# fgnt/pb_chime5

Measured on AMD Instinct MI355X. Metric: utterance-seconds enhanced/sec/GPU (24ch, 20 EM iters), higher is better.
Workload: dtype f64

## Files before the change

pb_chime5_amd/csrc/cacgmm.hip:

```cpp
#include <algorithm>
#include <cmath>
#include <cstdlib>

#include "gss_internal.h"
#include "dense_wave.h"
#include "jacobi.h"

namespace {

#ifndef GSS_CHOL_PRIO
#define GSS_CHOL_PRIO 1
#endif
#ifndef GSS_ESTEP_PRIO
#define GSS_ESTEP_PRIO 1
#endif
constexpr int EM_TILE = 64;
constexpr int EM_TS = EM_TILE + 1;

enum { MODE_FIRST = 0, MODE_EM = 1, MODE_PREDICT = 2 };

__device__ __forceinline__ void set_progress_priority(int done, int total) {
    const int q4 = 4 * done / total;
    if (q4 <= 0) __builtin_amdgcn_s_setprio(3);
    else if (q4 == 1) __builtin_amdgcn_s_setprio(2);
    else if (q4 == 2) __builtin_amdgcn_s_setprio(1);
    else __builtin_amdgcn_s_setprio(0);
}

struct MsegPlan {
    int S, ntile, base, rem, maxseg;
};
__host__ __device__ __forceinline__ int mseg_begin(const MsegPlan &p, int slot) {
    return slot * p.base + (slot < p.rem ? slot : p.rem);
}
__host__ __device__ __forceinline__ int mseg_slot_of(const MsegPlan &p, int item) {
    const int head = p.rem * (p.base + 1);
    return item < head ? item / (p.base + 1) : p.rem + (item - head) / p.base;
}
__host__ __device__ __forceinline__ int mseg_count(const MsegPlan &p, int f) {
    return mseg_slot_of(p, f * p.ntile + p.ntile - 1) - mseg_slot_of(p, f * p.ntile) + 1;
}

struct EmArgs {
    const cplx *Y;
    const uint8_t *act;
    int64_t act_stride, act_fstride;
    const double *init;
    int64_t init_stride, init_fstride;
    const double *logdet;
    const double *pi;
// ... 2041 lines not shown
```

pb_chime5_amd/csrc/gss_api.hip:

```cpp
#include <cmath>
#include <cstdarg>
#include <cstdlib>
#include <cstring>
#include <mutex>

#include "gss_internal.h"

#define GSS_ENTER(ctx)                                   \
    if (!(ctx)) return GSS_ERR_INVALID;                  \
    GSS_HIP_CHECK((ctx), hipSetDevice((ctx)->device))
#define GSS_ENTER_VARIANTS(ctx) \
    GSS_ENTER(ctx);             \
    GSS_TRY(variant_refresh(ctx))
static int variant_refresh(gss_ctx *ctx);

static std::mutex g_error_lock;

int gss_fail(gss_ctx *ctx, int code, const char *fmt, ...) {
    char buf[1024];
    va_list ap;
    va_start(ap, fmt);
    vsnprintf(buf, sizeof(buf), fmt, ap);
    va_end(ap);
    if (ctx) {
        std::lock_guard<std::mutex> guard(g_error_lock);
        ctx->error = buf;
    }
    return code;
}

static thread_local std::string g_create_error;

namespace {
const char *const kVariantKeys[] = {
    "corr_ts", "corr_nw", "corr_blocked", "corr_p_tiles", "chol_diag_unfolded", "apply_ph",
    "apply_generic", "prof_detail", "corr_stg8", "corr_ksplit", "apply_gglobal", "wpe_halves",
    "em_wgs", "estep_wpb", "estep_lds", "mstep_prefetch_d", "mstep_tiled", "mstep_plan_min_d",
    "mstep_chunked", "mstep_slots", "force_eigh", "em_unfused", "em_l3_mb", "em_l3_fit_mb",
    "em_streams", "mstep_maxseg", "em4_cold_eigh", "mstep_generic"};
struct VariantTable {
    std::mutex lock;
    std::string text;
    bool parsed = false;
    std::map<std::string, int> values;
};
VariantTable &variant_table() {
    static VariantTable t;
    return t;
}
}

static int variant_refresh(gss_ctx *ctx) {
    const char *env = getenv("GSS_VARIANT");
    VariantTable &t = variant_table();
    std::lock_guard<std::mutex> guard(t.lock);
    if (t.parsed && t.text == (env ? env : "")) return GSS_OK;
    t.text = env ? env : "";
    t.parsed = true;
    t.values.clear();
// ... 1142 lines not shown
```

pb_chime5_amd/csrc/gss_internal.h:

```cpp
#pragma once
#include <hip/hip_runtime.h>

#include <cstdint>
#include <cstdio>
#include <map>
#include <string>
#include <vector>

#include "../../include/gss_hip.h"

typedef double2 cplx;

int gss_variant(const char *key, int dflt);
inline bool gss_variant_set(const char *key) { return gss_variant(key, 0) != 0; }

#if (defined(GSS_CORR_TRACE) || defined(GSS_WCOV_TRACE) || defined(GSS_EM4_TRACE) || \
     defined(GSS_CHOL_TRACE)) && !defined(GSS_EXPERIMENT_BUILD)
#error "trace instrumentation needs -DGSS_EXPERIMENT_BUILD=1 (tools/build_variant.sh)"
#endif

#define GSS_TINY 2.2250738585072014e-308

__device__ __forceinline__ cplx c_make(double r, double i) { return make_double2(r, i); }
__device__ __forceinline__ cplx c_add(cplx a, cplx b) { return make_double2(a.x + b.x, a.y + b.y); }
// ... 41 lines not shown
    const int lo = __builtin_amdgcn_update_dpp(0, (int)(unsigned)u, CTRL, ROW_MASK, BANK_MASK, true);
    const int hi = __builtin_amdgcn_update_dpp(0, (int)(unsigned)(u >> 32), CTRL, ROW_MASK, BANK_MASK, true);
    return __longlong_as_double(((unsigned long long)(unsigned)hi << 32) | (unsigned)lo);
}
__device__ __forceinline__ double wave_sum(double v) {
    double s = v + dpp_shifted<0x111, 0xf, 0xf>(v);
    s += dpp_shifted<0x112, 0xf, 0xf>(v);
    s += dpp_shifted<0x113, 0xf, 0xf>(v);
    s += dpp_shifted<0x114, 0xf, 0xe>(s);
    s += dpp_shifted<0x118, 0xf, 0xc>(s);
    s += dpp_shifted<0x142, 0xa, 0xf>(s);
    s += dpp_shifted<0x143, 0xc, 0xf>(s);
    const unsigned long long u = __double_as_longlong(s);
    const unsigned lo = __builtin_amdgcn_readlane((int)(unsigned)u, 63);
    const unsigned hi = __builtin_amdgcn_readlane((int)(unsigned)(u >> 32), 63);
    return __longlong_as_double(((unsigned long long)hi << 32) | lo);
}
__device__ __forceinline__ double wave_max(double v) {
#pragma unroll
    for (int o = 32; o > 0; o >>= 1) v = fmax(v, __shfl_xor(v, o, 64));
    return v;
}

__device__ __forceinline__ bool xcd_group_map(int nsub, int F, int &f, int &sub) {
    const int L = blockIdx.x;
    const int sg = L / (8 * nsub), rem = L - sg * 8 * nsub;
    sub = rem >> 3;
    f = sg * 8 + (rem & 7);
    return f < F;
}
static inline unsigned xcd_grid(int nsub, int F) { return (unsigned)(nsub * ((F + 7) / 8 * 8)); }

__host__ __device__ __forceinline__ int tri_index(int d1, int d2, int D) {
    return d1 * D - (d1 * (d1 - 1)) / 2 + (d2 - d1);
}
__host__ __device__ __forceinline__ int tri_count(int D) { return D * (D + 1) / 2; }

struct ProfEntry {
    std::string name;
    hipEvent_t start, stop;
};

struct gss_ctx {
    int device = 0;
    hipStream_t own_stream = nullptr;
    hipStream_t stream = nullptr;
// ... 139 lines not shown
```

pb_chime5_amd/csrc/wpe.hip:

```cpp
#include <algorithm>
#include <cmath>
#include <cstdlib>

#include "gss_internal.h"
#include <type_traits>
#include "dense_wave.h"

typedef double v4d __attribute__((ext_vector_type(4)));

namespace {

constexpr int POW_FRAMES = 256;
__global__ __launch_bounds__(POW_FRAMES) void wpe_power_kernel(const cplx *__restrict__ X,
                                                               int64_t T, int D, int psd_context,
                                                               double *__restrict__ raw,
                                                               double *__restrict__ w) {
    extern __shared__ __attribute__((aligned(16))) char smem[];
    double *ps = reinterpret_cast<double *>(smem);
    __shared__ double red[POW_FRAMES / 64];
    const int f = blockIdx.x, tid = threadIdx.x;
    const cplx *Xf = X + (int64_t)f * T * D;
    double *wout = w + (int64_t)f * T;
    double *wf = psd_context > 0 ? raw + (int64_t)f * T : wout;
    const int DP = D + 1;
    double mx = 0.0;
    for (int64_t t0 = 0; t0 < T; t0 += POW_FRAMES) {
        const int nfr = (int)min((int64_t)POW_FRAMES, T - t0);
        const int total = nfr * D;
        const cplx *src = Xf + t0 * D;
        __syncthreads();
        {
            constexpr int LB = 8;
            const int qf = POW_FRAMES / D, rf = POW_FRAMES - qf * D;
            int fr = tid / D, d = tid - fr * D;
            for (int base = tid; base < total; base += LB * POW_FRAMES) {
                cplx v[LB];
#pragma unroll
                for (int j = 0; j < LB; ++j) {
                    const int idx = base + j * POW_FRAMES;
                    v[j] = idx < total ? src[idx] : c_make(0.0, 0.0);
                }
#pragma unroll
                for (int j = 0; j < LB; ++j) {
                    if (base + j * POW_FRAMES < total) ps[fr * DP + d] = c_abs2(v[j]);
                    fr += qf;
                    d += rf;
                    if (d >= D) {
                        d -= D;
                        ++fr;
// ... 1036 lines not shown
                    }
                    nxim[it] = -xim[it];
#pragma unroll
                    for (int reg = 0; reg < 4; ++reg) {
                        const int rl = 16 * it + lk + 4 * reg, col = c0 + 16 * b + li;
                        if (rl < nb && col < D)
                            Z[(int64_t)(j0 + rl) * D + col] = c_make(xre[it][reg], xim[it][reg]);
                    }
                }
            }
            __syncthreads();
        }
    }
}

__global__ __launch_bounds__(256, 3) void chol_backsolve_kernel(const cplx *__restrict__ R,
                                                             cplx *__restrict__ P, int n, int D) {
    __shared__ cplx S[CH_NB * BS_LD];
    __shared__ cplx OP[BS_OPS];
    const int f = blockIdx.x;
    chol_backsolve_body(R + (int64_t)f * n * n, P + (int64_t)f * n * D, n, D, S, OP);
}

template <int TA, int NB, int NWV = 4, int WRAPS = 4, bool TAIL = true>
__global__ __launch_bounds__(64 * NWV) void wpe_apply_kernel(const cplx *__restrict__ Y,
                                                        const cplx *__restrict__ G, int F,
                                                        int64_t T, int D, int n, int c,
                                                        cplx *__restrict__ X) {
    constexpr int WAVE_FRAMES = 16 * TA, WG_FRAMES = NWV * WAVE_FRAMES;
    extern __shared__ __attribute__((aligned(16))) char smem[];
    cplx *S = reinterpret_cast<cplx *>(smem);
    const int DP = D | 1;
    int f, chunk;
    if (!xcd_group_map((int)((T + WG_FRAMES - 1) / WG_FRAMES), F, f, chunk)) return;
    const int64_t t0 = (int64_t)chunk * WG_FRAMES;
    const cplx *Yf = Y + (int64_t)f * T * D;
    const cplx *Gf = G + (int64_t)f * n * D;
    const int frames_lds = WG_FRAMES + c + 2;
    const int64_t fr0 = t0 - c;
    constexpr int PRE = 14, NT = 64 * NWV;
    const int total = frames_lds * D;
    for (int base = 0; base < total; base += NT * PRE) {
        cplx v[PRE];
#pragma unroll
        for (int j = 0; j < PRE; ++j) {
            const int idx = base + (int)threadIdx.x + NT * j;
            const int64_t fr = fr0 + idx / D;
            v[j] = c_make(0.0, 0.0);
            if (idx < total && fr >= 0 && fr < T) v[j] = Yf[fr0 * D + idx];
        }
#pragma unroll
        for (int j = 0; j < PRE; ++j) {
            const int idx = base + (int)threadIdx.x + NT * j;
            const int fl = idx / D, d = idx - fl * D;
            if (idx < total) S[fl * DP + d] = v[j];
        }
    }
    __syncthreads();
    const int wave = threadIdx.x >> 6, lane = threadIdx.x & 63;
    const int li = lane & 15, lk = lane >> 4;
    const int wf0 = wave * WAVE_FRAMES;
    if (t0 + wf0 >= T) return;
    v4d acc_re[TA][NB], acc_im[TA][NB], acc_t2[TA][NB];
#pragma unroll
    for (int a = 0; a < TA; ++a)
#pragma unroll
        for (int b = 0; b < NB; ++b) {
            acc_re[a][b] = (v4d){0.0, 0.0, 0.0, 0.0};
            acc_im[a][b] = (v4d){0.0, 0.0, 0.0, 0.0};
            acc_t2[a][b] = (v4d){0.0, 0.0, 0.0, 0.0};
        }
    const int ksteps = (n + 3) / 4;
    const int lds_last = frames_lds * DP - 1;
    int goff[NB], goff_max[NB];
#pragma unroll
    for (int b = 0; b < NB; ++b) {
        const int col = min(16 * b + li, D - 1);
        goff[b] = min(lk, n - 1) * D + col;
        goff_max[b] = (n - 1) * D + col;
    }
    auto load_g = [&](int, cplx (&g)[NB]) {
#pragma unroll
        for (int b = 0; b < NB; ++b) {
            g[b] = Gf[goff[b]];
            goff[b] = min(goff[b] + 4 * D, goff_max[b]);
        }
    };
    int rm = lk % D, lin = (lk / D) * DP + rm;
    int ubase[TA];
#pragma unroll
    for (int a = 0; a < TA; ++a) ubase[a] = (wf0 + 16 * a + li) * DP;
    auto load_u = [&](cplx (&u)[TA]) {
#pragma unroll
        for (int a = 0; a < TA; ++a) u[a] = S[min(ubase[a] + lin, lds_last)];
        rm += 4;
        lin += 4;
#pragma unroll
        for (int w = 0; w < WRAPS; ++w) {
            const bool wrap = rm >= D;
            rm -= wrap ? D : 0;
            lin += wrap ? DP - D : 0;
        }
    };
    auto step = [&](int ks, const cplx (&g)[NB], const cplx (&u)[TA]) {
        const bool ok = !TAIL || 4 * ks + lk < n;
        double ur[TA], ui[TA], gr[NB], gi[NB];
#pragma unroll
        for (int a = 0; a < TA; ++a) {
            ur[a] = ok ? u[a].x : 0.0;
            ui[a] = ok ? u[a].y : 0.0;
        }
#pragma unroll
        for (int b = 0; b < NB; ++b) {
            gr[b] = g[b].x;
            gi[b] = g[b].y;
        }
        double us[TA], gd[NB];
#pragma unroll
        for (int a = 0; a < TA; ++a) us[a] = ur[a] + ui[a];
#pragma unroll
        for (int b = 0; b < NB; ++b) gd[b] = gr[b] - gi[b];
#pragma unroll
        for (int a = 0; a < TA; ++a)
#pragma unroll
            for (int b = 0; b < NB; ++b) {
                acc_re[a][b] = __builtin_amdgcn_mfma_f64_16x16x4f64(ur[a], gr[b], acc_re[a][b], 0, 0, 0);
                acc_t2[a][b] = __builtin_amdgcn_mfma_f64_16x16x4f64(ui[a], gi[b], acc_t2[a][b], 0, 0, 0);
                acc_im[a][b] = __builtin_amdgcn_mfma_f64_16x16x4f64(us[a], gd[b], acc_im[a][b], 0, 0, 0);
            }
    };
    cplx g0[NB], g1[NB], u0[TA], u1[TA];
    load_g(0, g0);
    load_u(u0);
    for (int ks = 0; ks < ksteps; ks += 2) {
        load_g(ks + 1, g1);
        load_u(u1);
        __builtin_amdgcn_sched_barrier(0);
        step(ks, g0, u0);
        __builtin_amdgcn_sched_barrier(0);
        load_g(ks + 2, g0);
        load_u(u0);
        __builtin_amdgcn_sched_barrier(0);
        step(ks + 1, g1, u1);
        __builtin_amdgcn_sched_barrier(0);
    }
#pragma unroll
    for (int a = 0; a < TA; ++a)
#pragma unroll
        for (int b = 0; b < NB; ++b)
#pragma unroll
            for (int reg = 0; reg < 4; ++reg) {
                const int fl = wf0 + 16 * a + lk + 4 * reg;
                const int d = 16 * b + li;
                const int64_t t = t0 + fl;
                if (d < D && t < T) {
                    const cplx y = S[(fl + c) * DP + d];
                    const double pre = acc_re[a][b][reg] + acc_t2[a][b][reg];
                    const double pim = (acc_im[a][b][reg] - acc_re[a][b][reg]) + acc_t2[a][b][reg];
                    X[((int64_t)f * T + t) * D + d] = c_make(y.x - pre, y.y - pim);
                }
            }
}

template <int PH, int NT, bool GLDS = true, int PREW = 14, int PREG = 14>
__global__ __launch_bounds__(256) void wpe_apply_packed_kernel(const cplx *__restrict__ Y,
                                                               const cplx *__restrict__ G, int F,
                                                               int64_t T, int D, int n, int c,
                                                               cplx *__restrict__ X) {
    constexpr int WG_ROWS = 64, WG_FRAMES = PH * WG_ROWS;
    extern __shared__ __attribute__((aligned(16))) char smem[];
    const int DP = D | 1, DG = GLDS ? (D | 1) : D;
    const int frames_lds = WG_FRAMES + c + 2;
    cplx *S = reinterpret_cast<cplx *>(smem);
    cplx *Gl = S + (frames_lds * DP + frames_lds / PH + 1);
    int f, chunk;
    if (!xcd_group_map((int)((T + WG_FRAMES - 1) / WG_FRAMES), F, f, chunk)) return;
    const int64_t t0 = (int64_t)chunk * WG_FRAMES;
    const cplx *Yf = Y + (int64_t)f * T * D;
    const cplx *Gf = G + (int64_t)f * n * D;
    const int64_t fr0 = t0 - c;
    constexpr int NTHR = 256;
    {
        constexpr int PRE = PREW;
        const int total = frames_lds * D;
// ... 304 lines not shown
static int corr_tiles_pairs(int n, int D, int c, std::vector<CorrTile> &tiles) {
    for (int r0 = 0; r0 < n; r0 += 16)
        for (int c0 = r0; c0 < n; c0 += 32) tiles.push_back({r0, c0, 0, c0 + 16 < n ? 3 : 1});
    for (int r0 = 0; r0 < n; r0 += 32)
        for (int c0 = 0; c0 < D; c0 += 16) tiles.push_back({r0, c * D + c0, 1, r0 + 16 < n ? 5 : 1});
    std::stable_sort(tiles.begin(), tiles.end(), [](const CorrTile &x, const CorrTile &y) {
        return __builtin_popcount(x.mask) > __builtin_popcount(y.mask);
    });
    return (int)tiles.size();
}

static int corr_padf(int D, int ct) { return (ct + D - 1) / D + 1; }

size_t wpe_workspace_bytes(int F, int64_t T, int D, int taps, int delay) {
    const size_t n = (size_t)taps * D;
    size_t b = 0;
    b += 2 * align_up(sizeof(double) * (size_t)F * T);
    b += align_up(sizeof(cplx) * (size_t)F * n * n);
    b += align_up(sizeof(cplx) * (size_t)F * n * D);
    return b + 4096;
}

static int wpe_power_launch(gss_ctx *ctx, const cplx *cur, int F, int64_t T, int D,
                            int psd_context, double *raw, double *w) {
    const size_t pow_lds = sizeof(double) * POW_FRAMES * (D + 1);
    if (pow_lds > 64 * 1024)
        GSS_HIP_CHECK(ctx, hipFuncSetAttribute(reinterpret_cast<const void *>(wpe_power_kernel),
                                               hipFuncAttributeMaxDynamicSharedMemorySize,
                                               (int)pow_lds));
    hipLaunchKernelGGL(wpe_power_kernel, dim3(F), dim3(POW_FRAMES), pow_lds, ctx->stream,
                       cur, T, D, psd_context, raw, w);
    GSS_LAUNCH_CHECK(ctx, "wpe_power_kernel");
    return GSS_OK;
}

int wpe_inverse_power_run(gss_ctx *ctx, const cplx *Y, int F, int64_t T, int D, int psd_context,
                          double *w) {
    double *raw = psd_context > 0 ? arena_alloc_t<double>(ctx, (size_t)F * T) : nullptr;
    GSS_REQUIRE(ctx, raw || psd_context == 0, GSS_ERR_NOMEM, "wpe power workspace");
    return wpe_power_launch(ctx, Y, F, T, D, psd_context, raw, w);
}

int wpe_run(gss_ctx *ctx, const cplx *Y, int F, int64_t T, int D, int taps, int delay,
            int iterations, int psd_context, cplx *X, int part, int array_bins) {
    const int n = taps * D;
    const int c = delay + taps - 1;
    if (iterations == 0) {
        GSS_HIP_CHECK(ctx, hipMemsetAsync(ctx->status_dev + 2, 0, sizeof(int32_t), ctx->stream));
        if (X != Y)
            GSS_HIP_CHECK(ctx, hipMemcpyAsync(X, Y, sizeof(cplx) * (size_t)F * T * D,
                                              hipMemcpyDeviceToDevice, ctx->stream));
        return GSS_OK;
    }
    GSS_REQUIRE(ctx, X != Y, GSS_ERR_INVALID, "gss_wpe: X must not alias Y");
    double *w = arena_alloc_t<double>(ctx, (size_t)F * T);
    double *raw = psd_context > 0 ? arena_alloc_t<double>(ctx, (size_t)F * T) : nullptr;
    cplx *R = arena_alloc_t<cplx>(ctx, (size_t)F * n * n);
    cplx *P = arena_alloc_t<cplx>(ctx, (size_t)F * n * D);
    GSS_REQUIRE(ctx, w && (raw || psd_context == 0) && R && P, GSS_ERR_NOMEM, "wpe workspace");

    std::vector<CorrTile> tiles;
    const int sub16 = (n + 15) / 16;
    int corr_ts = sub16 * (sub16 + 1) / 2 + sub16 * ((D + 15) / 16) <= CORR_FINE_MAX_SUBTILES ? 1 : 2;
    bool corr_pairs = false;
    if (const int e = gss_variant("corr_ts", 0)) {
        corr_ts = e == 1 ? 1 : 2;
        corr_pairs = e == 3;
    }
    const int ntiles = corr_pairs ? corr_tiles_pairs(n, D, c, tiles) : corr_tiles(n, D, c, 16 * corr_ts, tiles);
    constexpr int tm16 = 16, tn16 = 16;
    std::vector<UpdTile> upd;
    std::vector<int> upd_start, upd_count, upd_j0, upd_k, upd_ndiag;
    const bool fold_diag = !gss_variant_set("chol_diag_unfolded");
    {
        const int nblk = (n + CH_NB - 1) / CH_NB;
        for (int J = 0; J < nblk; ++J) {
            upd_start.push_back((int)upd.size());
            const int rs = (J + 1) * CH_NB;
            const bool narrow = J % 2 == 0;
            const int r_end = narrow ? std::min(rs + CH_NB, n) : n;
            const int d_end = std::min(rs + CH_NB, n);
            for (int r0 = rs; r0 < d_end; r0 += tm16)
// ... 55 lines not shown
                   : corr_ts == 1 ? (corr_nw == 2 ? wpe_corr_kernel<1, 2> : wpe_corr_kernel<1, 4>)
                                  : (corr_nw == 2 ? wpe_corr_kernel<2, 2> : wpe_corr_kernel<2, 4>);
    size_t corr_lds = sizeof(cplx) * (size_t)(CORR_KT + c + padf) * D + sizeof(double) * CORR_KT;
    const int ksplit_forced = gss_variant("corr_ksplit", 0);
    int cus = 0;
    if (array_bins > 0)
        GSS_HIP_CHECK(ctx, hipDeviceGetAttribute(&cus, hipDeviceAttributeMultiprocessorCount, ctx->device));
    const bool arrays_single_waves = array_bins > 0 && (int64_t)ntiles * array_bins >= 4LL * 16 * cus;
    const bool corr_split = ksplit_forced ? ksplit_forced != 1 : !arrays_single_waves;
    const int corr_ks = (corr_ts == 1 && corr_nw == 1 && corr_split)
                            ? (ksplit_forced == 2 ? 2 : 4) : 1;
    using corr_fn_t = void (*)(const cplx *, const double *, int, int64_t, int, int, int, int,
                               const CorrTile *, int, cplx *, cplx *);
    corr_fn_t ksplit_fn = nullptr;
    if (corr_ks > 1) {
        ksplit_fn = corr_stg5 ? (corr_ks == 2 ? wpe_corr_ksplit_kernel<2, 5> : wpe_corr_ksplit_kernel<4, 5>)
                              : (corr_ks == 2 ? wpe_corr_ksplit_kernel<2, 8> : wpe_corr_ksplit_kernel<4, 8>);
        corr_lds = std::max(corr_lds * corr_ks, sizeof(cplx) * 256 * (size_t)(corr_ks - 1));
    }
    const size_t panel_lds = sizeof(cplx) * UDP_SIZE + sizeof(double) * CH_NB;
    constexpr int apply_ta = 2;
    constexpr int apply_nwv = 4;
    const int apply_frames = 16 * apply_ta * apply_nwv;
    auto apply_fn = D <= 16 ? wpe_apply_kernel<apply_ta, 1> : wpe_apply_kernel<apply_ta, 2>;
    if (D >= 4 && !gss_variant_set("apply_generic")) {
        if (n % 8 == 0)
            apply_fn = D <= 16 ? wpe_apply_kernel<apply_ta, 1, 4, 1, false>
                               : wpe_apply_kernel<apply_ta, 2, 4, 1, false>;
        else
            apply_fn = D <= 16 ? wpe_apply_kernel<apply_ta, 1, 4, 1, true>
                               : wpe_apply_kernel<apply_ta, 2, 4, 1, true>;
    }
    const size_t apply_lds = sizeof(cplx) * (size_t)(apply_frames + c + 2) * (D | 1);
    int apply_ph = 1, apply_nt = (D + 15) / 16;
    size_t packed_lds = 0;
    {
        const int ph_env = gss_variant("apply_ph", 0);
        bool ph_env_taken = ph_env <= 1;
        double best = (double)((D + 15) / 16) * n;
        for (int ph = 2; ph <= 4; ++ph) {
            if (ph_env > 0 && ph != ph_env) continue;
            const int nt = (ph * D + 15) / 16;
            if (nt > 3 || D < 2) continue;
            const double cost = (double)nt * (n + (ph - 1) * D) / ph;
            const int fl = 64 * ph + c + 2;
            const size_t lds = sizeof(cplx) * ((size_t)fl * (D | 1) + fl / ph + 1 + (size_t)(n + 1) * (D | 1));
            if (lds > (ph_env == ph ? 160 : 64) * 1024) continue;
            if (cost < 0.75 * best || ph_env == ph) {
                ph_env_taken = ph_env_taken || ph_env == ph;
                best = cost;
                apply_ph = ph;
                apply_nt = nt;
                packed_lds = lds;
            }
        }
// ... 18 lines not shown
        packed_lds = sizeof(cplx) * ((size_t)fl * (D | 1) + fl / 2 + 1);
        packed_fn = wpe_apply_packed_kernel<2, 3, false>;
    } else
    if (apply_ph > 1) {
        static const apply_packed_t table[3][3] = {
            {wpe_apply_packed_kernel<2, 1>, wpe_apply_packed_kernel<2, 2>, wpe_apply_packed_kernel<2, 3>},
            {wpe_apply_packed_kernel<3, 1>, wpe_apply_packed_kernel<3, 2>, wpe_apply_packed_kernel<3, 3>},
            {wpe_apply_packed_kernel<4, 1>, wpe_apply_packed_kernel<4, 2>, wpe_apply_packed_kernel<4, 3>}};
        packed_fn = table[apply_ph - 2][apply_nt - 1];
        static const apply_packed_t table_small[3][3] = {
            {wpe_apply_packed_kernel<2, 1, true, 4, 1>, wpe_apply_packed_kernel<2, 2, true, 4, 1>, wpe_apply_packed_kernel<2, 3, true, 4, 1>},
            {wpe_apply_packed_kernel<3, 1, true, 4, 1>, wpe_apply_packed_kernel<3, 2, true, 4, 1>, wpe_apply_packed_kernel<3, 3, true, 4, 1>},
            {wpe_apply_packed_kernel<4, 1, true, 4, 1>, wpe_apply_packed_kernel<4, 2, true, 4, 1>, wpe_apply_packed_kernel<4, 3, true, 4, 1>}};
        if ((64 * apply_ph + c + 2) * D <= 4 * 256 && n * D <= 256 && !gss_variant_set("apply_generic"))
            packed_fn = table_small[apply_ph - 2][apply_nt - 1];
        if (packed_lds > 64 * 1024)
            GSS_HIP_CHECK(ctx, hipFuncSetAttribute(reinterpret_cast<const void *>(packed_fn),
                                                   hipFuncAttributeMaxDynamicSharedMemorySize,
                                                   (int)packed_lds));
    }
    GSS_REQUIRE(ctx, corr_lds <= 160 * 1024 && apply_lds <= 160 * 1024, GSS_ERR_UNSUPPORTED,
                "wpe: taps=%d D=%d needs more LDS than a CU has", taps, D);
    if (apply_lds > 64 * 1024)
        GSS_HIP_CHECK(ctx, hipFuncSetAttribute(reinterpret_cast<const void *>(apply_fn),
                                               hipFuncAttributeMaxDynamicSharedMemorySize,
                                               (int)apply_lds));
    if (corr_lds > 64 * 1024)
        GSS_HIP_CHECK(ctx, hipFuncSetAttribute(reinterpret_cast<const void *>(corr_fn),
                                               hipFuncAttributeMaxDynamicSharedMemorySize,
                                               (int)corr_lds));
    const int corr_pieces = (int)(((size_t)(CORR_KT + c + padf) * D + 63) / 64);
    const size_t corr_dma_lds = 2 * (sizeof(cplx) * 64 * (size_t)corr_pieces + sizeof(double) * CORR_KT);
    const bool corr_persist = corr_ts == 2 && (int64_t)T * D * 16 < (1LL << 31) &&
                              corr_dma_lds <= 80 * 1024;
    if (corr_persist && !nw_forced) corr_nw = 4;
    const bool corr_blocked = corr_persist && gss_variant_set("corr_blocked");
    auto corr_persist_fn = corr_blocked ? (corr_nw == 2 ? wpe_corr_persist_kernel<2, true>
                                                        : wpe_corr_persist_kernel<4, true>)
                                        : (corr_nw == 2 ? wpe_corr_persist_kernel<2>
                                                        : wpe_corr_persist_kernel<4>);
    CorrQueue corr_queue{(ntiles + corr_nw - 1) / corr_nw, 0};
    int corr_slots = 0;
    if (corr_persist) {
        for (int g = 0; g < corr_queue.ngroups; ++g)
            if (__builtin_popcount(tiles[g * corr_nw].mask) >= 3) corr_queue.gh = g + 1;
        if (corr_dma_lds > 64 * 1024)
            GSS_HIP_CHECK(ctx, hipFuncSetAttribute(reinterpret_cast<const void *>(corr_persist_fn),
                                                   hipFuncAttributeMaxDynamicSharedMemorySize,
                                                   (int)corr_dma_lds));
        int per_cu = 0, cus = 0;
        GSS_HIP_CHECK(ctx, hipOccupancyMaxActiveBlocksPerMultiprocessor(
                               &per_cu, reinterpret_cast<const void *>(corr_persist_fn), 64 * corr_nw,
                               corr_dma_lds));
        GSS_HIP_CHECK(ctx, hipDeviceGetAttribute(&cus, hipDeviceAttributeMultiprocessorCount, ctx->device));
        corr_slots = std::min(std::max(per_cu, 1) * cus, corr_queue.ngroups * F);
    }

    for (int it = 0; it < iterations; ++it) {
        const cplx *cur = it == 0 ? Y : X;
        {
            GSS_PROF(ctx, "wpe_power");
            GSS_TRY(wpe_power_launch(ctx, cur, F, T, D, psd_context, raw, w));
        }
        if (corr_persist) {
            GSS_HIP_CHECK(ctx, hipMemsetAsync(corr_counters, 0, 8 * 16 * sizeof(int), ctx->stream));
            GSS_PROF(ctx, "wpe_corr");
            hipLaunchKernelGGL(corr_persist_fn, dim3(corr_slots), dim3(64 * corr_nw), corr_dma_lds,
                               ctx->stream, Y, w, F, T, D, n, c, corr_pieces, tiles_dev, ntiles,
                               corr_queue, corr_counters, R, P);
            GSS_LAUNCH_CHECK(ctx, "wpe_corr_persist_kernel");
        } else {
            GSS_PROF(ctx, "wpe_corr");
            if (ksplit_fn)
                hipLaunchKernelGGL(ksplit_fn, dim3(xcd_grid(ntiles, F)), dim3(64 * corr_ks), corr_lds,
                                   ctx->stream, Y, w, F, T, D, n, c, padf, tiles_dev, ntiles, R, P);
            else
                hipLaunchKernelGGL(corr_fn, dim3(xcd_grid((ntiles + corr_nw - 1) / corr_nw, F)),
                                   dim3(64 * corr_nw), corr_lds,
                                   ctx->stream, Y, w, F, T, D, n, c, padf, tiles_dev, ntiles, R, P);
            GSS_LAUNCH_CHECK(ctx, "wpe_corr_kernel");
        }
        {
            const int nblk = (n + CH_NB - 1) / CH_NB;
            const bool detail = gss_variant_set("prof_detail");
            static const char *trsm_names[] = {"wpe_chol_trsm_J0", "wpe_chol_trsm_J1", "wpe_chol_trsm_J2",
// ... 21 lines not shown
                    const int ndiag = upd_ndiag[J];
                    const dim3 g((ndiag > 0 ? (F + 7) / 8 * 8 : 0) +
                                 xcd_grid((nupd - ndiag + UPD_WAVES - 1) / UPD_WAVES, F)), b(64 * UPD_WAVES);
                    const UpdTile *tl = upd_dev + upd_start[J];
                    hipLaunchKernelGGL((chol_update_kernel<1, 1, true>), g, b, 0, ctx->stream, R, P, F, n, D, upd_j0[J],
                                       std::min(upd_k[J], n - upd_j0[J]), tl, nupd, ndiag,
                                       (J + 1) * CH_NB, zero_pivots);
                    GSS_LAUNCH_CHECK(ctx, "chol_update_kernel");
                }
            }
            {
                GSS_PROF(ctx, "wpe_backsolve");
                hipLaunchKernelGGL(chol_backsolve_kernel, dim3(F), dim3(256), 0, ctx->stream, R, P, n,
                                   D);
                GSS_LAUNCH_CHECK(ctx, "chol_backsolve_kernel");
            }
        }
        {
            GSS_PROF(ctx, "wpe_apply");
            if (packed_fn) {
                const int wg_frames = 64 * apply_ph;
                hipLaunchKernelGGL(packed_fn, dim3(xcd_grid((int)((T + wg_frames - 1) / wg_frames), F)),
                                   dim3(256), packed_lds, ctx->stream, Y, P, F, T, D, n, c, X);
            } else {
                hipLaunchKernelGGL(apply_fn,
                                   dim3(xcd_grid((int)((T + apply_frames - 1) / apply_frames), F)),
                                   dim3(64 * apply_nwv), apply_lds, ctx->stream, Y, P, F, T, D, n, c, X);
            }
            GSS_LAUNCH_CHECK(ctx, "wpe_apply_kernel");
        }
    }
    if (part < 0)
        GSS_HIP_CHECK(ctx, hipMemcpyAsync(ctx->status_host + 2, zero_pivots, sizeof(int32_t),
                                          hipMemcpyDeviceToHost, ctx->stream));
    return GSS_OK;
}


int wpe_copy_zero_pivots(gss_ctx *ctx) {
    if (!ctx->wpe_tiles) return GSS_OK;
    const int32_t *zero_pivots =
        reinterpret_cast<const int32_t *>(reinterpret_cast<const CorrTile *>(ctx->wpe_tiles) + 1024 + 4096);
    GSS_HIP_CHECK(ctx, hipMemcpyAsync(ctx->status_host + 2, zero_pivots, sizeof(int32_t),
                                      hipMemcpyDeviceToHost, ctx->stream));
    return GSS_OK;
}

int selftest_mfma_run(gss_ctx *ctx) {
    double *out = nullptr;
    GSS_HIP_CHECK(ctx, hipMalloc(reinterpret_cast<void **>(&out), sizeof(double) * 256));
// ... 17 lines not shown
```

Before: 1091.

## Fuse WPE power computation into apply kernel and add persistent run-based apply

```diff
diff --git a/pb_chime5_amd/csrc/cacgmm.hip b/pb_chime5_amd/csrc/cacgmm.hip
--- a/pb_chime5_amd/csrc/cacgmm.hip
+++ b/pb_chime5_amd/csrc/cacgmm.hip
@@ -18,14 +18,6 @@
 constexpr int EM_TS = EM_TILE + 1;
 
 enum { MODE_FIRST = 0, MODE_EM = 1, MODE_PREDICT = 2 };
-
-__device__ __forceinline__ void set_progress_priority(int done, int total) {
-    const int q4 = 4 * done / total;
-    if (q4 <= 0) __builtin_amdgcn_s_setprio(3);
-    else if (q4 == 1) __builtin_amdgcn_s_setprio(2);
-    else if (q4 == 2) __builtin_amdgcn_s_setprio(1);
-    else __builtin_amdgcn_s_setprio(0);
-}
 
 struct MsegPlan {
     int S, ntile, base, rem, maxseg;
diff --git a/pb_chime5_amd/csrc/gss_api.hip b/pb_chime5_amd/csrc/gss_api.hip
--- a/pb_chime5_amd/csrc/gss_api.hip
+++ b/pb_chime5_amd/csrc/gss_api.hip
@@ -35,6 +35,7 @@
 const char *const kVariantKeys[] = {
     "corr_ts", "corr_nw", "corr_blocked", "corr_p_tiles", "chol_diag_unfolded", "apply_ph",
     "apply_generic", "prof_detail", "corr_stg8", "corr_ksplit", "apply_gglobal", "wpe_halves",
+    "power_pass", "apply_grid",
     "em_wgs", "estep_wpb", "estep_lds", "mstep_prefetch_d", "mstep_tiled", "mstep_plan_min_d",
     "mstep_chunked", "mstep_slots", "force_eigh", "em_unfused", "em_l3_mb", "em_l3_fit_mb",
     "em_streams", "mstep_maxseg", "em4_cold_eigh", "mstep_generic"};
diff --git a/pb_chime5_amd/csrc/gss_internal.h b/pb_chime5_amd/csrc/gss_internal.h
--- a/pb_chime5_amd/csrc/gss_internal.h
+++ b/pb_chime5_amd/csrc/gss_internal.h
@@ -87,6 +87,20 @@
     return v;
 }
 
+__device__ __forceinline__ void set_progress_priority(int done, int total) {
+    const int q4 = 4 * done / total;
+    if (q4 <= 0) __builtin_amdgcn_s_setprio(3);
+    else if (q4 == 1) __builtin_amdgcn_s_setprio(2);
+    else if (q4 == 2) __builtin_amdgcn_s_setprio(1);
+    else __builtin_amdgcn_s_setprio(0);
+}
+
+__device__ __forceinline__ void wave_lds_sync() {
+    __builtin_amdgcn_fence(__ATOMIC_RELEASE, "wavefront");
+    __builtin_amdgcn_wave_barrier();
+    __builtin_amdgcn_fence(__ATOMIC_ACQUIRE, "wavefront");
+}
+
 __device__ __forceinline__ bool xcd_group_map(int nsub, int F, int &f, int &sub) {
     const int L = blockIdx.x;
     const int sg = L / (8 * nsub), rem = L - sg * 8 * nsub;
diff --git a/pb_chime5_amd/csrc/wpe.hip b/pb_chime5_amd/csrc/wpe.hip
--- a/pb_chime5_amd/csrc/wpe.hip
+++ b/pb_chime5_amd/csrc/wpe.hip
@@ -11,6 +11,7 @@
 namespace {
 
 constexpr int POW_FRAMES = 256;
+template <bool FROM_RAW = false>
 __global__ __launch_bounds__(POW_FRAMES) void wpe_power_kernel(const cplx *__restrict__ X,
                                                                int64_t T, int D, int psd_context,
                                                                double *__restrict__ raw,
@@ -21,10 +22,17 @@
     const int f = blockIdx.x, tid = threadIdx.x;
     const cplx *Xf = X + (int64_t)f * T * D;
     double *wout = w + (int64_t)f * T;
-    double *wf = psd_context > 0 ? raw + (int64_t)f * T : wout;
+    double *wf = psd_context > 0 || FROM_RAW ? raw + (int64_t)f * T : wout;
     const int DP = D + 1;
     double mx = 0.0;
-    for (int64_t t0 = 0; t0 < T; t0 += POW_FRAMES) {
+    if (FROM_RAW && psd_context == 0) {
+        for (int64_t t = tid; t < T; t += POW_FRAMES) {
+            const double p = wf[t];
+            wout[t] = p;
+            mx = fmax(mx, p);
+        }
+    }
+    for (int64_t t0 = 0; !FROM_RAW && t0 < T; t0 += POW_FRAMES) {
         const int nfr = (int)min((int64_t)POW_FRAMES, T - t0);
         const int total = nfr * D;
         const cplx *src = Xf + t0 * D;
@@ -1107,11 +1115,147 @@
     chol_backsolve_body(R + (int64_t)f * n * n, P + (int64_t)f * n * D, n, D, S, OP);
 }
 
-template <int TA, int NB, int NWV = 4, int WRAPS = 4, bool TAIL = true>
+template <int TA, int NB, int WRAPS, bool TAIL, bool POWER, bool SHARED>
+__device__ __forceinline__ void apply_wave_tile(const cplx *S, double *Q, int frames_lds, int wf0,
+                                                bool active, const cplx *__restrict__ Gf, int f,
+                                                int64_t t0, int64_t T, int D, int DP, int n, int c,
+                                                cplx *__restrict__ X, double *__restrict__ raw,
+                                                int lane) {
+    constexpr int WAVE_FRAMES = 16 * TA;
+    const int li = lane & 15, lk = lane >> 4;
+    v4d acc_re[TA][NB], acc_im[TA][NB], acc_t2[TA][NB];
+#pragma unroll
+    for (int a = 0; a < TA; ++a)
+#pragma unroll
+        for (int b = 0; b < NB; ++b) {
+            acc_re[a][b] = (v4d){0.0, 0.0, 0.0, 0.0};
+            acc_im[a][b] = (v4d){0.0, 0.0, 0.0, 0.0};
+            acc_t2[a][b] = (v4d){0.0, 0.0, 0.0, 0.0};
+        }
+    const int ksteps = active ? (n + 3) / 4 : 0;
+    const int lds_last = frames_lds * DP - 1;
+    int goff[NB], goff_max[NB];
+#pragma unroll
+    for (int b = 0; b < NB; ++b) {
+        const int col = min(16 * b + li, D - 1);
+        goff[b] = min(lk, n - 1) * D + col;
+        goff_max[b] = (n - 1) * D + col;
+    }
+    auto load_g = [&](int, cplx (&g)[NB]) {
+#pragma unroll
+        for (int b = 0; b < NB; ++b) {
+            g[b] = Gf[goff[b]];
+            goff[b] = min(goff[b] + 4 * D, goff_max[b]);
+        }
+    };
+    int rm = lk % D, lin = (lk / D) * DP + rm;
+    int ubase[TA];
+#pragma unroll
+    for (int a = 0; a < TA; ++a) ubase[a] = (wf0 + 16 * a + li) * DP;
+    auto load_u = [&](cplx (&u)[TA]) {
+#pragma unroll
+        for (int a = 0; a < TA; ++a) u[a] = S[min(ubase[a] + lin, lds_last)];
+        rm += 4;
+        lin += 4;
+#pragma unroll
+        for (int w = 0; w < WRAPS; ++w) {
+            const bool wrap = rm >= D;
+            rm -= wrap ? D : 0;
+            lin += wrap ? DP - D : 0;
+        }
+    };
+    auto step = [&](int ks, const cplx (&g)[NB], const cplx (&u)[TA]) {
+        const bool ok = !TAIL || 4 * ks + lk < n;
+        double ur[TA], ui[TA], gr[NB], gi[NB];
+#pragma unroll
+        for (int a = 0; a < TA; ++a) {
+            ur[a] = ok ? u[a].x : 0.0;
+            ui[a] = ok ? u[a].y : 0.0;
+        }
+#pragma unroll
+        for (int b = 0; b < NB; ++b) {
+            gr[b] = g[b].x;
+            gi[b] = g[b].y;
+        }
+        double us[TA], gd[NB];
+#pragma unroll
+        for (int a = 0; a < TA; ++a) us[a] = ur[a] + ui[a];
+#pragma unroll
+        for (int b = 0; b < NB; ++b) gd[b] = gr[b] - gi[b];
+#pragma unroll
+        for (int a = 0; a < TA; ++a)
+#pragma unroll
+            for (int b = 0; b < NB; ++b) {
+                acc_re[a][b] = __builtin_amdgcn_mfma_f64_16x16x4f64(ur[a], gr[b], acc_re[a][b], 0, 0, 0);
+                acc_t2[a][b] = __builtin_amdgcn_mfma_f64_16x16x4f64(ui[a], gi[b], acc_t2[a][b], 0, 0, 0);
+                acc_im[a][b] = __builtin_amdgcn_mfma_f64_16x16x4f64(us[a], gd[b], acc_im[a][b], 0, 0, 0);
+            }
+    };
+    cplx g0[NB], g1[NB], u0[TA], u1[TA];
+    load_g(0, g0);
+    load_u(u0);
+    for (int ks = 0; ks < ksteps; ks += 2) {
+        load_g(ks + 1, g1);
+        load_u(u1);
+        __builtin_amdgcn_sched_barrier(0);
+        step(ks, g0, u0);
+        __builtin_amdgcn_sched_barrier(0);
+        load_g(ks + 2, g0);
+        load_u(u0);
+        __builtin_amdgcn_sched_barrier(0);
+        step(ks + 1, g1, u1);
+        __builtin_amdgcn_sched_barrier(0);
+    }
+    double pw[TA][NB][4];
+#pragma unroll
+    for (int a = 0; a < TA; ++a)
+#pragma unroll
+        for (int b = 0; b < NB; ++b)
+#pragma unroll
+            for (int reg = 0; reg < 4; ++reg) {
+                const int fl = wf0 + 16 * a + lk + 4 * reg;
+                const int d = 16 * b + li;
+                const int64_t t = t0 + fl;
+                pw[a][b][reg] = 0.0;
+                if (d < D && t < T) {
+                    const cplx y = S[(fl + c) * DP + d];
+                    const double pre = acc_re[a][b][reg] + acc_t2[a][b][reg];
+                    const double pim = (acc_im[a][b][reg] - acc_re[a][b][reg]) + acc_t2[a][b][reg];
+                    const cplx x = c_make(y.x - pre, y.y - pim);
+                    if (POWER)
+                        pw[a][b][reg] = c_abs2(x);
+                    else
+                        X[((int64_t)f * T + t) * D + d] = x;
+                }
+            }
+    if (POWER) {
+        static_assert(WAVE_FRAMES <= 64, "one lane per frame of a wave");
+        if (SHARED) __syncthreads(); else wave_lds_sync();
+#pragma unroll
+        for (int a = 0; a < TA; ++a)
+#pragma unroll
+            for (int b = 0; b < NB; ++b)
+#pragma unroll
+                for (int reg = 0; reg < 4; ++reg) {
+                    const int d = 16 * b + li;
+                    if (d < D) Q[(16 * a + lk + 4 * reg) * DP + d] = pw[a][b][reg];
+                }
+        if (SHARED) __syncthreads(); else wave_lds_sync();
+        const int64_t t = t0 + wf0 + lane;
+        if (lane < WAVE_FRAMES && t < T) {
+            double p = 0.0;
+            for (int d = 0; d < D; ++d) p += Q[lane * DP + d];
+            raw[(int64_t)f * T + t] = p / (double)D;
+        }
+    }
+}
+
+template <int TA, int NB, int NWV = 4, int WRAPS = 4, bool TAIL = true, bool POWER = false>
 __global__ __launch_bounds__(64 * NWV) void wpe_apply_kernel(const cplx *__restrict__ Y,
                                                         const cplx *__restrict__ G, int F,
                                                         int64_t T, int D, int n, int c,
-                                                        cplx *__restrict__ X) {
+                                                        cplx *__restrict__ X,
+                                                        double *__restrict__ raw) {
     constexpr int WAVE_FRAMES = 16 * TA, WG_FRAMES = NWV * WAVE_FRAMES;
     extern __shared__ __attribute__((aligned(16))) char smem[];
     cplx *S = reinterpret_cast<cplx *>(smem);
@@ -1143,108 +1287,71 @@
     }
     __syncthreads();
     const int wave = threadIdx.x >> 6, lane = threadIdx.x & 63;
-    const int li = lane & 15, lk = lane >> 4;
     const int wf0 = wave * WAVE_FRAMES;
-    if (t0 + wf0 >= T) return;
-    v4d acc_re[TA][NB], acc_im[TA][NB], acc_t2[TA][NB];
-#pragma unroll
-    for (int a = 0; a < TA; ++a)
-#pragma unroll
-        for (int b = 0; b < NB; ++b) {
-            acc_re[a][b] = (v4d){0.0, 0.0, 0.0, 0.0};
-            acc_im[a][b] = (v4d){0.0, 0.0, 0.0, 0.0};
-            acc_t2[a][b] = (v4d){0.0, 0.0, 0.0, 0.0};
-        }
-    const int ksteps = (n + 3) / 4;
-    const int lds_last = frames_lds * DP - 1;
-    int goff[NB], goff_max[NB];
-#pragma unroll
-    for (int b = 0; b < NB; ++b) {
-        const int col = min(16 * b + li, D - 1);
-        goff[b] = min(lk, n - 1) * D + col;
-        goff_max[b] = (n - 1) * D + col;
-    }
-    auto load_g = [&](int, cplx (&g)[NB]) {
-#pragma unroll
-        for (int b = 0; b < NB; ++b) {
-            g[b] = Gf[goff[b]];
-            goff[b] = min(goff[b] + 4 * D, goff_max[b]);
-        }
-    };
-    int rm = lk % D, lin = (lk / D) * DP + rm;
-    int ubase[TA];
-#pragma unroll
-    for (int a = 0; a < TA; ++a) ubase[a] = (wf0 + 16 * a + li) * DP;
-    auto load_u = [&](cplx (&u)[TA]) {
-#pragma unroll
-        for (int a = 0; a < TA; ++a) u[a] = S[min(ubase[a] + lin, lds_last)];
-        rm += 4;
-        lin += 4;
-#pragma unroll
-        for (int w = 0; w < WRAPS; ++w) {
-            const bool wrap = rm >= D;
-            rm -= wrap ? D : 0;
-            lin += wrap ? DP - D : 0;
-        }
-    };
-    auto step = [&](int ks, const cplx (&g)[NB], const cplx (&u)[TA]) {
-        const bool ok = !TAIL || 4 * ks + lk < n;
-        double ur[TA], ui[TA], gr[NB], gi[NB];
-#pragma unroll
-        for (int a = 0; a < TA; ++a) {
-            ur[a] = ok ? u[a].x : 0.0;
-            ui[a] = ok ? u[a].y : 0.0;
-        }
-#pragma unroll
-        for (int b = 0; b < NB; ++b) {
-            gr[b] = g[b].x;
-            gi[b] = g[b].y;
-        }
-        double us[TA], gd[NB];
-#pragma unroll
-        for (int a = 0; a < TA; ++a) us[a] = ur[a] + ui[a];
-#pragma unroll
-        for (int b = 0; b < NB; ++b) gd[b] = gr[b] - gi[b];
-#pragma unroll
-        for (int a = 0; a < TA; ++a)
-#pragma unroll
-            for (int b = 0; b < NB; ++b) {
-                acc_re[a][b] = __builtin_amdgcn_mfma_f64_16x16x4f64(ur[a], gr[b], acc_re[a][b], 0, 0, 0);
-                acc_t2[a][b] = __builtin_amdgcn_mfma_f64_16x16x4f64(ui[a], gi[b], acc_t2[a][b], 0, 0, 0);
-                acc_im[a][b] = __builtin_amdgcn_mfma_f64_16x16x4f64(us[a], gd[b], acc_im[a][b], 0, 0, 0);
-            }
-    };
-    cplx g0[NB], g1[NB], u0[TA], u1[TA];
-    load_g(0, g0);
-    load_u(u0);
-    for (int ks = 0; ks < ksteps; ks += 2) {
-        load_g(ks + 1, g1);
-        load_u(u1);
-        __builtin_amdgcn_sched_barrier(0);
-        step(ks, g0, u0);
-        __builtin_amdgcn_sched_barrier(0);
-        load_g(ks + 2, g0);
-        load_u(u0);
-        __builtin_amdgcn_sched_barrier(0);
-        step(ks + 1, g1, u1);
-        __builtin_amdgcn_sched_barrier(0);
-    }
-#pragma unroll
-    for (int a = 0; a < TA; ++a)
-#pragma unroll
-        for (int b = 0; b < NB; ++b)
-#pragma unroll
-            for (int reg = 0; reg < 4; ++reg) {
-                const int fl = wf0 + 16 * a + lk + 4 * reg;
-                const int d = 16 * b + li;
-                const int64_t t = t0 + fl;
-                if (d < D && t < T) {
-                    const cplx y = S[(fl + c) * DP + d];
-                    const double pre = acc_re[a][b][reg] + acc_t2[a][b][reg];
-                    const double pim = (acc_im[a][b][reg] - acc_re[a][b][reg]) + acc_t2[a][b][reg];
-                    X[((int64_t)f * T + t) * D + d] = c_make(y.x - pre, y.y - pim);
+    const bool active = t0 + wf0 < T;
+    if (!POWER && !active) return;
+    apply_wave_tile<TA, NB, WRAPS, TAIL, POWER, true>(S, reinterpret_cast<double *>(smem) + wf0 * DP,
+                                                      frames_lds, wf0, active, Gf, f, t0, T, D, DP, n,
+                                                      c, X, raw, lane);
+}
+
+template <int TA, int NB, int NWV = 4, int WRAPS = 4, bool TAIL = true, bool POWER = false>
+__global__ __launch_bounds__(64 * NWV) void wpe_apply_runs_kernel(const cplx *__restrict__ Y,
+                                                             const cplx *__restrict__ G, int ntile,
+                                                             int nitems, int64_t T, int D, int n,
+                                                             int c, cplx *__restrict__ X,
+                                                             double *__restrict__ raw) {
+    constexpr int WAVE_FRAMES = 16 * TA;
+    extern __shared__ __attribute__((aligned(16))) char smem[];
+    const int DP = D | 1;
+    const int wave = __builtin_amdgcn_readfirstlane((int)threadIdx.x >> 6), lane = threadIdx.x & 63;
+    const int frames_lds = WAVE_FRAMES + c + 2;
+    cplx *S = reinterpret_cast<cplx *>(smem) + wave * frames_lds * DP;
+    const int nwaves = (int)gridDim.x * NWV, w = (int)blockIdx.x * NWV + wave;
+    const int run = nitems / nwaves, rem = nitems - run * nwaves;
+    const int beg = w * run + min(w, rem), end = beg + run + (w < rem ? 1 : 0);
+    const int total = frames_lds * D;
+    const int qf = 64 / D, rf = 64 - qf * D;
+    const int fl0 = lane / D, d0 = lane - fl0 * D;
+    int f = beg / ntile, tile = beg - f * ntile;
+    for (int item = beg; item < end; ++item) {
+        set_progress_priority(item - beg, end - beg);
+        const int64_t t0 = (int64_t)tile * WAVE_FRAMES;
+        const int64_t fr0 = t0 - c;
+        const cplx *src = Y + ((int64_t)f * T + fr0) * D;
+        constexpr int PRE = NB == 1 ? 6 : 18;
+        int fl = fl0, d = d0;
+        for (int base = 0; base < total; base += 64 * PRE) {
+            cplx v[PRE];
+            int so[PRE];
+#pragma unroll
+            for (int j = 0; j < PRE; ++j) {
+                const int idx = base + lane + 64 * j;
+                const int64_t fr = fr0 + fl;
+                v[j] = c_make(0.0, 0.0);
+                if (idx < total && fr >= 0 && fr < T) v[j] = src[idx];
+                so[j] = idx < total ? fl * DP + d : -1;
+                fl += qf;
+                d += rf;
+                if (d >= D) {
+                    d -= D;
+                    ++fl;
                 }
             }
+#pragma unroll
+            for (int j = 0; j < PRE; ++j)
+                if (so[j] >= 0) S[so[j]] = v[j];
+        }
+        wave_lds_sync();
+        apply_wave_tile<TA, NB, WRAPS, TAIL, POWER, false>(S, reinterpret_cast<double *>(S), frames_lds,
+                                                           0, true, G + (int64_t)f * n * D, f, t0, T,
+                                                           D, DP, n, c, X, raw, lane);
+        wave_lds_sync();
+        if (++tile == ntile) {
+            tile = 0;
+            ++f;
+        }
+    }
 }
 
 template <int PH, int NT, bool GLDS = true, int PREW = 14, int PREG = 14>
@@ -1595,13 +1702,19 @@
 }
 
 static int wpe_power_launch(gss_ctx *ctx, const cplx *cur, int F, int64_t T, int D,
-                            int psd_context, double *raw, double *w) {
+                            int psd_context, double *raw, double *w, bool from_raw = false) {
+    if (from_raw) {
+        hipLaunchKernelGGL(wpe_power_kernel<true>, dim3(F), dim3(POW_FRAMES), 0, ctx->stream,
+                           cur, T, D, psd_context, raw, w);
+        GSS_LAUNCH_CHECK(ctx, "wpe_power_kernel");
+        return GSS_OK;
+    }
     const size_t pow_lds = sizeof(double) * POW_FRAMES * (D + 1);
     if (pow_lds > 64 * 1024)
-        GSS_HIP_CHECK(ctx, hipFuncSetAttribute(reinterpret_cast<const void *>(wpe_power_kernel),
+        GSS_HIP_CHECK(ctx, hipFuncSetAttribute(reinterpret_cast<const void *>(wpe_power_kernel<false>),
                                                hipFuncAttributeMaxDynamicSharedMemorySize,
                                                (int)pow_lds));
-    hipLaunchKernelGGL(wpe_power_kernel, dim3(F), dim3(POW_FRAMES), pow_lds, ctx->stream,
+    hipLaunchKernelGGL(wpe_power_kernel<false>, dim3(F), dim3(POW_FRAMES), pow_lds, ctx->stream,
                        cur, T, D, psd_context, raw, w);
     GSS_LAUNCH_CHECK(ctx, "wpe_power_kernel");
     return GSS_OK;
@@ -1612,6 +1725,31 @@
     double *raw = psd_context > 0 ? arena_alloc_t<double>(ctx, (size_t)F * T) : nullptr;
     GSS_REQUIRE(ctx, raw || psd_context == 0, GSS_ERR_NOMEM, "wpe power workspace");
     return wpe_power_launch(ctx, Y, F, T, D, psd_context, raw, w);
+}
+
+using apply_fn_t = void (*)(const cplx *, const cplx *, int, int64_t, int, int, int, cplx *, double *);
+template <int TA, bool POWER>
+static apply_fn_t pick_apply(int D, int form) {
+    if (form == 1)
+        return D <= 16 ? wpe_apply_kernel<TA, 1, 4, 1, false, POWER> : wpe_apply_kernel<TA, 2, 4, 1, false, POWER>;
+    if (form == 2)
+        return D <= 16 ? wpe_apply_kernel<TA, 1, 4, 1, true, POWER> : wpe_apply_kernel<TA, 2, 4, 1, true, POWER>;
+    return D <= 16 ? wpe_apply_kernel<TA, 1, 4, 4, true, POWER> : wpe_apply_kernel<TA, 2, 4, 4, true, POWER>;
+}
+
+constexpr int kApplyGridDefault = 1;
+using apply_runs_fn_t = void (*)(const cplx *, const cplx *, int, int, int64_t, int, int, int, cplx *,
+                                 double *);
+template <int TA, bool POWER>
+static apply_runs_fn_t pick_apply_runs(int D, int form) {
+    if (form == 1)
+        return D <= 16 ? wpe_apply_runs_kernel<TA, 1, 4, 1, false, POWER>
+                       : wpe_apply_runs_kernel<TA, 2, 4, 1, false, POWER>;
+    if (form == 2)
+        return D <= 16 ? wpe_apply_runs_kernel<TA, 1, 4, 1, true, POWER>
+                       : wpe_apply_runs_kernel<TA, 2, 4, 1, true, POWER>;
+    return D <= 16 ? wpe_apply_runs_kernel<TA, 1, 4, 4, true, POWER>
+                   : wpe_apply_runs_kernel<TA, 2, 4, 4, true, POWER>;
 }
 
 int wpe_run(gss_ctx *ctx, const cplx *Y, int F, int64_t T, int D, int taps, int delay,
@@ -1627,10 +1765,11 @@
     }
     GSS_REQUIRE(ctx, X != Y, GSS_ERR_INVALID, "gss_wpe: X must not alias Y");
     double *w = arena_alloc_t<double>(ctx, (size_t)F * T);
-    double *raw = psd_context > 0 ? arena_alloc_t<double>(ctx, (size_t)F * T) : nullptr;
+    double *raw = psd_context > 0 || iterations > 1 ? arena_alloc_t<double>(ctx, (size_t)F * T) : nullptr;
     cplx *R = arena_alloc_t<cplx>(ctx, (size_t)F * n * n);
     cplx *P = arena_alloc_t<cplx>(ctx, (size_t)F * n * D);
-    GSS_REQUIRE(ctx, w && (raw || psd_context == 0) && R && P, GSS_ERR_NOMEM, "wpe workspace");
+    GSS_REQUIRE(ctx, w && (raw || (psd_context == 0 && iterations <= 1)) && R && P, GSS_ERR_NOMEM,
+                "wpe workspace");
 
     std::vector<CorrTile> tiles;
     const int sub16 = (n + 15) / 16;
@@ -1732,15 +1871,9 @@
     constexpr int apply_ta = 2;
     constexpr int apply_nwv = 4;
     const int apply_frames = 16 * apply_ta * apply_nwv;
-    auto apply_fn = D <= 16 ? wpe_apply_kernel<apply_ta, 1> : wpe_apply_kernel<apply_ta, 2>;
-    if (D >= 4 && !gss_variant_set("apply_generic")) {
-        if (n % 8 == 0)
-            apply_fn = D <= 16 ? wpe_apply_kernel<apply_ta, 1, 4, 1, false>
-                               : wpe_apply_kernel<apply_ta, 2, 4, 1, false>;
-        else
-            apply_fn = D <= 16 ? wpe_apply_kernel<apply_ta, 1, 4, 1, true>
-                               : wpe_apply_kernel<apply_ta, 2, 4, 1, true>;
-    }
+    const int apply_form = !(D >= 4 && !gss_variant_set("apply_generic")) ? 0 : n % 8 == 0 ? 1 : 2;
+    auto apply_fn = pick_apply<apply_ta, false>(D, apply_form);
+    auto apply_power_fn = pick_apply<apply_ta, true>(D, apply_form);
     const size_t apply_lds = sizeof(cplx) * (size_t)(apply_frames + c + 2) * (D | 1);
     int apply_ph = 1, apply_nt = (D + 15) / 16;
     size_t packed_lds = 0;
@@ -1805,9 +1938,35 @@
     GSS_REQUIRE(ctx, corr_lds <= 160 * 1024 && apply_lds <= 160 * 1024, GSS_ERR_UNSUPPORTED,
                 "wpe: taps=%d D=%d needs more LDS than a CU has", taps, D);
     if (apply_lds > 64 * 1024)
-        GSS_HIP_CHECK(ctx, hipFuncSetAttribute(reinterpret_cast<const void *>(apply_fn),
-                                               hipFuncAttributeMaxDynamicSharedMemorySize,
-                                               (int)apply_lds));
+        for (apply_fn_t fn : {apply_fn, apply_power_fn})
+            GSS_HIP_CHECK(ctx, hipFuncSetAttribute(reinterpret_cast<const void *>(fn),
+                                                   hipFuncAttributeMaxDynamicSharedMemorySize,
+                                                   (int)apply_lds));
+    const bool fuse_power = !packed_fn && iterations > 1 && !gss_variant_set("power_pass");
+    const int apply_ntile = (int)((T + 16 * apply_ta - 1) / (16 * apply_ta));
+    const size_t runs_lds = sizeof(cplx) * (size_t)apply_nwv * (16 * apply_ta + c + 2) * (D | 1);
+    const bool apply_runs = !packed_fn && 2 * runs_lds <= 160 * 1024 &&
+                            (int64_t)F * apply_ntile < (1LL << 31) &&
+                            gss_variant("apply_grid", kApplyGridDefault) == 0;
+    apply_runs_fn_t runs_fn[2] = {pick_apply_runs<apply_ta, false>(D, apply_form),
+                                  pick_apply_runs<apply_ta, true>(D, apply_form)};
+    int runs_grid[2] = {0, 0};
+    if (apply_runs) {
+        int cus = 0;
+        GSS_HIP_CHECK(ctx, hipDeviceGetAttribute(&cus, hipDeviceAttributeMultiprocessorCount, ctx->device));
+        const int nitems = F * apply_ntile;
+        for (int i = 0; i < 2; ++i) {
+            if (runs_lds > 64 * 1024)
+                GSS_HIP_CHECK(ctx, hipFuncSetAttribute(reinterpret_cast<const void *>(runs_fn[i]),
+                                                       hipFuncAttributeMaxDynamicSharedMemorySize,
+                                                       (int)runs_lds));
+            int per_cu = 0;
+            GSS_HIP_CHECK(ctx, hipOccupancyMaxActiveBlocksPerMultiprocessor(
+                                   &per_cu, reinterpret_cast<const void *>(runs_fn[i]), 64 * apply_nwv,
+                                   runs_lds));
+            runs_grid[i] = std::min(std::max(per_cu, 1) * cus, (nitems + apply_nwv - 1) / apply_nwv);
+        }
+    }
     if (corr_lds > 64 * 1024)
         GSS_HIP_CHECK(ctx, hipFuncSetAttribute(reinterpret_cast<const void *>(corr_fn),
                                                hipFuncAttributeMaxDynamicSharedMemorySize,
@@ -1843,7 +2002,7 @@
         const cplx *cur = it == 0 ? Y : X;
         {
             GSS_PROF(ctx, "wpe_power");
-            GSS_TRY(wpe_power_launch(ctx, cur, F, T, D, psd_context, raw, w));
+            GSS_TRY(wpe_power_launch(ctx, cur, F, T, D, psd_context, raw, w, fuse_power && it > 0));
         }
         if (corr_persist) {
             GSS_HIP_CHECK(ctx, hipMemsetAsync(corr_counters, 0, 8 * 16 * sizeof(int), ctx->stream));
@@ -1911,10 +2070,15 @@
                 const int wg_frames = 64 * apply_ph;
                 hipLaunchKernelGGL(packed_fn, dim3(xcd_grid((int)((T + wg_frames - 1) / wg_frames), F)),
                                    dim3(256), packed_lds, ctx->stream, Y, P, F, T, D, n, c, X);
+            } else if (apply_runs) {
+                const int pw = fuse_power && it + 1 < iterations ? 1 : 0;
+                hipLaunchKernelGGL(runs_fn[pw], dim3(runs_grid[pw]), dim3(64 * apply_nwv), runs_lds,
+                                   ctx->stream, Y, P, apply_ntile, F * apply_ntile, T, D, n, c, X, raw);
             } else {
-                hipLaunchKernelGGL(apply_fn,
+                hipLaunchKernelGGL(fuse_power && it + 1 < iterations ? apply_power_fn : apply_fn,
                                    dim3(xcd_grid((int)((T + apply_frames - 1) / apply_frames), F)),
-                                   dim3(64 * apply_nwv), apply_lds, ctx->stream, Y, P, F, T, D, n, c, X);
+                                   dim3(64 * apply_nwv), apply_lds, ctx->stream, Y, P, F, T, D, n, c, X,
+                                   raw);
             }
             GSS_LAUNCH_CHECK(ctx, "wpe_apply_kernel");
         }
```

Result: no change. 1095, median of 6 (+0.3%).
